# whwh747/A-Low-Texture-Robust-Hybrid-Feature-Based-Visual-Odometry

Hardware: AMD Instinct MI355X
Metric: RGB-D frames/sec (640×480, 1k ORB + LSD + PEAC) at 1/2/4/8 GPUs (higher is better)
Workload: dtype u8/u16 integer + f32/f64; 1 GPU; 640x480 synthetic RGB-D, 1000 ORB (quota; 3/4 std + 1/4 lowtex scenes) + LSD lines + PEAC planes, 8192 frames per GPU per step (std640); frames_per_gpu=8192, parallelism=frames sharded, 1 rank(s), no data-path collective, distinct_frames=256, resident_bytes_per_frame_estimate=21100000

## Files before the change

a-low-texture-robust-hybrid-feature-based-visual-odometry_amd/csrc/hvo_internal.hpp:

```cpp
#pragma once
#include <hip/hip_runtime.h>
#include <stdlib.h>
#include <stdint.h>
#include <string>
#include <vector>
#include "../../include/hvo.h"

#define HVO_MAX_LEVELS 16
#define HVO_EDGE_THRESHOLD 19
#define HVO_CELL_TILE 72
#define HVO_CELL_CAP 256
#define HVO_MAX_PROFILE 768
#define HVO_HAVE_PEAC 1
#define HVO_HAVE_LSD 1

struct LevelGeom {
    int w, h, pitch;
    int minBX, minBY, maxBX, maxBY;
    int nCols, nRows, wCell, hCell;
    int cell_off, ncells;
    int nfeat;
    int cand_off, cand_cap;
    int node_off, node_cap;
    int kp_off, kp_cap;
    int scaled_patch;
    float scale;
    unsigned long long img_off;
    unsigned long long lvl_off;
    int rs_off;
    int ry_off;
    int tile_off, ntx, nty;
};

struct CellDesc {
    short level, x0, y0, vw, vh, ox, oy, pad;
};

struct OrbTile {
    short bx0, by0, bw, bh;
    short fx0, fw;
    short cell;
    short dxa, dxb, dya, dyb;
    short pad[5];
};

struct OrbPlan {
    int w = 0, h = 0, nlevels = 0, batch = 0;
    LevelGeom lev[HVO_MAX_LEVELS];
    int ncells = 0, cand_total = 0, node_total = 0, kp_total = 0, ntiles = 0, max_cell = 0;
    size_t pyr_bytes = 0;
    size_t lvl_bytes = 0, blur_bytes = 0;
    int chunk = 0;
    bool resize_dw[HVO_MAX_LEVELS] = {};
    int last_chunks = 0;
    bool fused = false;
    int lt_off[HVO_MAX_LEVELS] = {}, lt_cnt[HVO_MAX_LEVELS] = {}, lt_tpw = 4;
    int lt_nw = 4;
    OrbTile *d_ltiles = nullptr;
    int2 *d_kpchunks = nullptr; int n_kpchunks = 0;
    int kp_cap = 0;
    LevelGeom *d_lev = nullptr;
    CellDesc *d_cells = nullptr;
    int *d_rs_xofs = nullptr; int *d_rs_xalpha = nullptr;
    int *d_rs_yofs = nullptr; int *d_rs_ybeta = nullptr;
    int4 *d_tiles = nullptr;
    uint8_t *d_pyr = nullptr, *d_blur = nullptr;
    uint8_t *d_lvl = nullptr, *d_lvl_base = nullptr;
    uint8_t *d_pyr_base = nullptr;
    uint32_t *d_cell_kp = nullptr; int *d_cell_cnt = nullptr;
    uint32_t *d_cand = nullptr; int *d_keys = nullptr, *d_keys_tmp = nullptr;
    int oct_slot_cap = 0;
    uint32_t *d_lvl_kp = nullptr; int *d_lvl_cnt = nullptr;
    hvo_keypoint *d_kp = nullptr; uint8_t *d_desc = nullptr; int *d_nkp = nullptr;
    int *d_flags = nullptr;
};

struct ProfileRec { const char *name; hipEvent_t e0, e1; float ms; bool used; hipStream_t st; };

struct Knob {
    bool set = false; int v = 0;
    void read(const char *name) { const char *e = getenv(name); set = e != nullptr; v = e ? atoi(e) : 0; }
    int or_(int dflt) const { return set ? v : dflt; }
    bool off() const { return set && v == 0; }
};
int hvo_ensure_dyn_lds(const void *kernel, size_t bytes);

struct hvo_ctx {
    hvo_params p;
    Knob kn_frame_perm, kn_upload_single;
    unsigned readings = 0;
    int device = 0;
    hipStream_t stream = nullptr;
    hipStream_t s_lsd = nullptr;
    hipStream_t s_peac = nullptr;
    hipEvent_t ev_lsd_pre = nullptr;
    bool lsd_pre_recorded = false;
    hipEvent_t ev_fast = nullptr;
    bool fast_recorded = false;
    int sched = 1;
    int sched_cfg = -1;
    bool orb_blur_late = false;
    uint8_t *d_stage_gray = nullptr; uint16_t *d_stage_depth = nullptr; size_t stage_gray_bytes = 0, stage_depth_bytes = 0;
    uint8_t *stage_gray_dst = nullptr; uint16_t *stage_depth_dst = nullptr;
    int stage_n = 0, stage_w = 0, stage_h = 0; bool stage_depth = false;
    hipStream_t s_stage_up = nullptr, s_stage_down = nullptr; hipEvent_t ev_stage_up = nullptr;
    char *d_result_slab = nullptr; size_t result_slab_bytes = 0;
    hipStream_t s_copy = nullptr; bool copy_hi = false;
    std::vector<std::pair<int, int *>> perms;
    double cull_dis = 5.0, cull_angle = 2.5, cull_endpoint = 15.0;
    bool last_cull = false;
    unsigned last_stages = 0;
    std::string last_error;
    OrbPlan orb;
    int umax[16];
    float scale[HVO_MAX_LEVELS], inv_scale[HVO_MAX_LEVELS];
    int nfeat[HVO_MAX_LEVELS];
    int8_t *d_pattern = nullptr; int *d_umax = nullptr;
    int batch_n = 0, batch_w = 0, batch_h = 0;
    bool have_depth = false;
    void *marena = nullptr;
    void *h_stage = nullptr; size_t h_stage_cap = 0;
    hipEvent_t ev_stage[2] = { nullptr, nullptr };
    bool profile = false;
    bool serialize = false;
    bool lsd_on_orb_stream = false;
    ProfileRec prof[HVO_MAX_PROFILE]; int nprof = 0;
    void *call_arena = nullptr; size_t call_arena_cap = 0;
    hipEvent_t po_ev[2] = { nullptr, nullptr }; float po_ms = 0.f;
    hipEvent_t ls_ev[3] = { nullptr, nullptr, nullptr }; float ls_ms[2] = { 0.f, 0.f };
    bool ls_batch_done = false;
    void *tail = nullptr;
    void *peac = nullptr;
    void *lsd = nullptr;
};

struct EdgeSel { unsigned s0, s1, s2; bool lo2; };
#ifdef __HIPCC__
static __device__ __forceinline__ EdgeSel edge_sel(int x0, int w)
{
    EdgeSel e; e.s0 = 0x03020100u; e.s1 = 0x07060504u; e.s2 = 0x07060504u;
    const int m = w - 1 - x0;
    e.lo2 = m <= 2;
    if (x0 >= 4 && m >= 7) return e;
    unsigned s0 = 0, s1 = 0, s2 = 0;
#pragma unroll
    for (int b = 0; b < 12; b++) {
        const int px = x0 - 4 + b;
        int r = px < 0 ? -px : (px >= w ? 2 * (w - 1) - px : px);
        int sb = r - (x0 - 4);
        if (b < 8) { if (sb < 0 || sb > 7) sb = b; }
        else if (e.lo2) { if (sb < 0 || sb > 7) sb = 7; }
        else { sb -= 4; if (sb < 0 || sb > 7) sb = b - 4; }
        if (b < 4) s0 |= (unsigned)sb << (8 * b);
        else if (b < 8) s1 |= (unsigned)sb << (8 * (b - 4));
        else s2 |= (unsigned)sb << (8 * (b - 8));
    }
    e.s0 = s0; e.s1 = s1; e.s2 = s2;
    return e;
}
static __device__ __forceinline__ void edge_fix(const EdgeSel &e, unsigned &W0, unsigned &W1, unsigned &W2)
{
    const unsigned a = e.lo2 ? W1 : W2, b = e.lo2 ? W0 : W1;
    const unsigned n0 = __builtin_amdgcn_perm(W1, W0, e.s0), n1 = __builtin_amdgcn_perm(W1, W0, e.s1);
    W2 = __builtin_amdgcn_perm(a, b, e.s2); W0 = n0; W1 = n1;
}
#endif

#define HVO_HIP(call)                                                                        \
    do {                                                                                     \
        hipError_t e_ = (call);                                                              \
        if (e_ != hipSuccess) {                                                              \
            ctx->last_error = std::string(#call) + ": " + hipGetErrorString(e_);            \
            return HVO_ERR_HIP;                                                              \
        }                                                                                    \
    } while (0)

static __device__ __forceinline__ double hvo_div_const(double a, double b, double y)
{
    const double q0 = a * y;
    const double q1 = fma(fma(-q0, b, a), y, q0);
    return fma(fma(-q1, b, a), y, q1);
}

static __device__ __forceinline__ float hvo_fatan2_deg(float y, float x)
{
    const float p1 = 0.9997878412794807f * (float)(180 / 3.14159265358979323846);
    const float p3 = -0.3258083974640975f * (float)(180 / 3.14159265358979323846);
    const float p5 = 0.1555786518463281f * (float)(180 / 3.14159265358979323846);
    const float p7 = -0.04432655554792128f * (float)(180 / 3.14159265358979323846);
    const float eps = (float)2.2204460492503131e-16;
    const float ax = fabsf(x), ay = fabsf(y);
    const bool hi = ax >= ay;
    const float c = __fdiv_rn(hi ? ay : ax, __fadd_rn(hi ? ax : ay, eps)), c2 = __fmul_rn(c, c);
    float r = __fmul_rn(__fadd_rn(__fmul_rn(__fadd_rn(__fmul_rn(__fadd_rn(__fmul_rn(p7, c2), p5), c2), p3), c2), p1), c);
    if (!hi) r = __fsub_rn(90.f, r);
    if (x < 0) r = __fsub_rn(180.f, r);
    if (y < 0) r = __fsub_rn(360.f, r);
// ... 201 lines not shown
```

a-low-texture-robust-hybrid-feature-based-visual-odometry_amd/csrc/orb_level.hip:

```cpp
#include "hvo_internal.hpp"
#include <string.h>
#include <algorithm>
#include <vector>

#define LT_TP 64
#define LT_ND (LT_TP / 4)
#define LT_TR 46
#define LT_MAXO 40
#define LT_CAND 368
#define LT_PEND 328
#define LT_TABN 48

typedef unsigned short lt_us2 __attribute__((ext_vector_type(2)));

struct __attribute__((aligned(16))) LtWave {
    uint32_t T[LT_TR * LT_ND];
    union {
        struct { uint8_t S[LT_TR * LT_TP]; unsigned short cand[LT_CAND]; unsigned short pend[LT_PEND]; unsigned long long mk_min[8], mk_ini[8]; } f;
        uint32_t V[((LT_TR + 1) / 2) * LT_MAXO];
    } u;
    int tab[4][LT_TABN];
};
static_assert(sizeof(LtWave) <= 8192, "five workgroups per CU");

struct LevelArgs {
    const uint8_t *rd; size_t rd_stride;
    uint8_t *wr; size_t wr_stride;
    uint8_t *blur; size_t blur_stride;
    LevelGeom L, D; int has_next;
    const OrbTile *tiles; int ntiles, tpw, groups, nframes;
    const int *xofs, *xalpha, *yofs, *ybeta;
    uint32_t *cell_kp; int *cell_cnt; int ncells, iniTh, minTh; int *flags;
    int k0, k1, k2, k3;
    int res_dw;
    int skip;
};

static __device__ __forceinline__ int lt_reflect(int p, int n)
{
    if (p < 0) p = -p;
    if (p >= n) p = 2 * (n - 1) - p;
    return p < 0 ? 0 : p;
}
static __device__ __forceinline__ int lt_mbcnt(unsigned long long m)
{
    return __builtin_amdgcn_mbcnt_hi((unsigned)(m >> 32), __builtin_amdgcn_mbcnt_lo((unsigned)m, 0u));
}

static __device__ __forceinline__ int lt_min3(int a, int b, int c) { int r; asm("v_min3_i32 %0, %1, %2, %3" : "=v"(r) : "v"(a), "v"(b), "v"(c)); return r; }
static __device__ __forceinline__ int lt_max3(int a, int b, int c) { int r; asm("v_max3_i32 %0, %1, %2, %3" : "=v"(r) : "v"(a), "v"(b), "v"(c)); return r; }

static __device__ __forceinline__ int lt_fast_score(const uint8_t *p, int v)
{
    constexpr int tp = LT_TP;
    int r[16];
    r[0] = p[3 * tp];    r[1] = p[3 * tp + 1];   r[2] = p[2 * tp + 2];   r[3] = p[tp + 3];
    r[4] = p[3];         r[5] = p[-tp + 3];      r[6] = p[-2 * tp + 2];  r[7] = p[-3 * tp + 1];
    r[8] = p[-3 * tp];   r[9] = p[-3 * tp - 1];  r[10] = p[-2 * tp - 2]; r[11] = p[-tp - 3];
    r[12] = p[-3];       r[13] = p[tp - 3];      r[14] = p[2 * tp - 2];  r[15] = p[3 * tp - 1];
    int d[16], e[16], a3[16], b3[16];
#pragma unroll
    for (int k = 0; k < 16; k++) { d[k] = v - r[k]; e[k] = r[k] - v; }
#pragma unroll
    for (int k = 0; k < 16; k++) { a3[k] = lt_min3(d[k], d[(k + 1) & 15], d[(k + 2) & 15]); b3[k] = lt_min3(e[k], e[(k + 1) & 15], e[(k + 2) & 15]); }
    int best = -1000;
#pragma unroll
    for (int k = 0; k < 16; k++)
        best = lt_max3(best, lt_min3(a3[k], a3[(k + 3) & 15], a3[(k + 6) & 15]), lt_min3(b3[k], b3[(k + 3) & 15], b3[(k + 6) & 15]));
    return best - 1;
}

static __device__ __forceinline__ void lt_row_sums(unsigned W0, unsigned W1, unsigned W2, unsigned klo, unsigned khi, unsigned hs[4])
{
    const unsigned A0 = __builtin_amdgcn_alignbyte(W1, W0, 1), B0 = __builtin_amdgcn_alignbyte(W2, W1, 1);
    const unsigned A1 = __builtin_amdgcn_alignbyte(W1, W0, 2), B1 = __builtin_amdgcn_alignbyte(W2, W1, 2);
    const unsigned A2 = __builtin_amdgcn_alignbyte(W1, W0, 3), B2 = __builtin_amdgcn_alignbyte(W2, W1, 3);
    hs[0] = __builtin_amdgcn_udot4(A0, klo, __builtin_amdgcn_udot4(B0, khi, 0u, false), false);
    hs[1] = __builtin_amdgcn_udot4(A1, klo, __builtin_amdgcn_udot4(B1, khi, 0u, false), false);
    hs[2] = __builtin_amdgcn_udot4(A2, klo, __builtin_amdgcn_udot4(B2, khi, 0u, false), false);
    hs[3] = __builtin_amdgcn_udot4(W1, klo, __builtin_amdgcn_udot4(W2, khi, 0u, false), false);
}
static __device__ __forceinline__ unsigned lt_dot2(unsigned a, unsigned w, unsigned c)
{
    return __builtin_amdgcn_udot2(__builtin_bit_cast(lt_us2, a), __builtin_bit_cast(lt_us2, w), c, false);
}

template <int NW>
__global__ __launch_bounds__(64 * NW, 5) void k_orb_level(const LevelArgs A)
{
    __shared__ LtWave lds_[NW];
    const int wv = threadIdx.x >> 6, lane = threadIdx.x & 63;
    const int xcd = blockIdx.x & 7, q = blockIdx.x >> 3;
    const int fr8 = q / A.groups, g = q - fr8 * A.groups;
    const int frame = fr8 * 8 + xcd;
    if (frame >= A.nframes) return;
    LtWave &W = lds_[wv];
    const LevelGeom &L = A.L;
    const uint8_t *img = A.rd + (size_t)frame * A.rd_stride;
    uint8_t *bdst = A.blur + (size_t)frame * A.blur_stride;
    const uint8_t *T8 = reinterpret_cast<const uint8_t *>(W.T);
    const unsigned long long ltm = (1ull << lane) - 1ull;

    for (int ti = 0; ti < A.tpw; ti++) {
        const int tidx = (g * A.tpw + ti) * NW + wv;
        if (tidx >= A.ntiles) break;
        const OrbTile t = A.tiles[tidx];
        const int lx0 = t.bx0 - 4, ly0 = t.by0 - 3;
        const int rows = t.bh + 6;
        const int xr = max(t.fx0 + t.fw, t.bx0 + t.bw) + 3;
        __builtin_amdgcn_wave_barrier();
        {
            typedef uint32_t lt_u4 __attribute__((ext_vector_type(4), aligned(4)));
            uint4 v[3];
#pragma unroll
            for (int k = 0; k < 3; k++) {
                const int i = lane + 64 * k, r = i >> 2, c = i & 3;
                v[k] = make_uint4(0, 0, 0, 0);
                if (r < rows) {
                    const int y = lt_reflect(ly0 + r, L.h);
                    const lt_u4 q4 = *reinterpret_cast<const lt_u4 *>(img + (size_t)y * L.pitch + lx0 + 16 * c);
                    v[k] = make_uint4(q4.x, q4.y, q4.z, q4.w);
                }
            }
            int tb0 = 0, tb1 = 0, tb2 = 0, tb3 = 0;
            const bool want_tab = A.has_next && lane < LT_TABN;
            if (want_tab) {
                const int dx = min(t.dxa + lane, A.D.w - 1), dy = min(t.dya + lane, A.D.h - 1);
                tb0 = A.xofs[dx]; tb1 = A.xalpha[dx]; tb2 = A.yofs[dy]; tb3 = A.ybeta[dy];
            }
#pragma unroll
            for (int k = 0; k < 3; k++) {
                const int i = lane + 64 * k;
                if ((i >> 2) < rows) reinterpret_cast<uint4 *>(W.T)[i] = v[k];
            }
            if (want_tab) { W.tab[0][lane] = tb0; W.tab[1][lane] = tb1; W.tab[2][lane] = tb2; W.tab[3][lane] = tb3; }
        }
        if (lx0 < 0) {
            if (lane < rows) { const unsigned d1 = W.T[lane * LT_ND + 1]; W.T[lane * LT_ND] = __builtin_amdgcn_perm(d1, d1, 0x01020300u); }
        }
        if (xr > L.w) {
            uint8_t *Tb = reinterpret_cast<uint8_t *>(W.T);
            if (lane < rows) {
                const int c = L.w - lx0;
#pragma unroll
                for (int k = 0; k < 3; k++) if (L.w + k < xr) Tb[lane * LT_TP + c + k] = Tb[lane * LT_TP + c - 2 - k];
            }
        }
        __builtin_amdgcn_wave_barrier();

        if (t.fw > 0 && !(A.skip & 1)) {
            uint8_t *S = W.u.f.S;
            {
                uint4 *Sz = reinterpret_cast<uint4 *>(S);
                const int nz = (rows * LT_TP + 15) >> 4;
                for (int i = lane; i < nz; i += 64) Sz[i] = make_uint4(0, 0, 0, 0);
            }
            const int cx0 = t.fx0 - lx0, cx1 = cx0 + t.fw, ih = t.bh, iw = t.fw, P = iw * ih;
            const int dws = cx0 >> 2, nd = ((cx1 - 1) >> 2) - dws + 1, items = ih * nd;
            const int rcp = (65536 + nd - 1) / nd;
            const int minTh = A.minTh;
            int ncand = 0, npend = 0;
            auto rest = [&](const unsigned short *pp, int cnt) {
                int pass = 0, xy = 0;
                if (lane < cnt) {
                    xy = pp[lane];
                    const uint8_t *qq = T8 + (xy >> 8) * LT_TP + (xy & 0xFF);
                    const int v = qq[0];
#define LT_PMN(o) min((int)qq[o], (int)qq[-(o)])
#define LT_PMX(o) max((int)qq[o], (int)qq[-(o)])
                    const int n0 = LT_PMN(3 * LT_TP), n1 = LT_PMN(3), n2 = LT_PMN(2 * LT_TP + 2), n3 = LT_PMN(-2 * LT_TP + 2);
                    const int n4 = LT_PMN(3 * LT_TP + 1), n5 = LT_PMN(LT_TP + 3), n6 = LT_PMN(-LT_TP + 3), n7 = LT_PMN(-3 * LT_TP + 1);
                    const int x0 = LT_PMX(3 * LT_TP), x1 = LT_PMX(3), x2 = LT_PMX(2 * LT_TP + 2), x3 = LT_PMX(-2 * LT_TP + 2);
                    const int x4 = LT_PMX(3 * LT_TP + 1), x5 = LT_PMX(LT_TP + 3), x6 = LT_PMX(-LT_TP + 3), x7 = LT_PMX(-3 * LT_TP + 1);
#undef LT_PMN
#undef LT_PMX
                    const int M1 = lt_max3(lt_max3(n0, n1, n2), lt_max3(n3, n4, n5), max(n6, n7));
                    const int M2 = lt_min3(lt_min3(x0, x1, x2), lt_min3(x3, x4, x5), min(x6, x7));
                    pass = (int)(M1 < v - minTh) | (int)(M2 > v + minTh);
                }
                const unsigned long long m = __ballot(pass != 0);
                const int p = ncand + __popcll(m & ltm);
                if (pass && p < LT_CAND) W.u.f.cand[p] = (unsigned short)xy;
                ncand += __popcll(m);
            };
            for (int base = 0; base < items; base += 64) {
                const int it = base + lane;
                const int ok = it < items;
                const int itc = ok ? it : 0;
                const int r = (itc * rcp) >> 16, dwi = dws + itc - r * nd;
                const unsigned t4 = W.T[r * LT_ND + dwi], v4 = W.T[(r + 3) * LT_ND + dwi], b4 = W.T[(r + 6) * LT_ND + dwi];
                const int xb = 4 * dwi;
                const int jl = max(cx0 - xb, 0), jh = min(cx1 - xb, 4);
                const unsigned inm = ok ? (((1u << jh) - 1u) & ~((1u << jl) - 1u)) : 0u;
                int pj[4];
#pragma unroll
                for (int j = 0; j < 4; j++) {
                    const int v = (v4 >> (8 * j)) & 0xFF, tt = (t4 >> (8 * j)) & 0xFF, bb = (b4 >> (8 * j)) & 0xFF;
                    pj[j] = (int)((inm >> j) & 1u) & ((int)(min(tt, bb) < v - minTh) | (int)(max(tt, bb) > v + minTh));
                }
                const unsigned long long m0 = __ballot(pj[0] != 0), m1 = __ballot(pj[1] != 0), m2 = __ballot(pj[2] != 0), m3 = __ballot(pj[3] != 0);
                if ((m0 | m1 | m2 | m3) != 0ull) {
                    const int p0 = npend + lt_mbcnt(m0) + lt_mbcnt(m1) + lt_mbcnt(m2) + lt_mbcnt(m3);
                    const int p1 = p0 + pj[0], p2 = p1 + pj[1], p3 = p2 + pj[2];
                    const int yx = ((r + 3) << 8) | xb;
                    W.u.f.pend[pj[0] ? p0 : LT_PEND - 1] = (unsigned short)yx;
                    W.u.f.pend[pj[1] ? p1 : LT_PEND - 1] = (unsigned short)(yx + 1);
                    W.u.f.pend[pj[2] ? p2 : LT_PEND - 1] = (unsigned short)(yx + 2);
                    W.u.f.pend[pj[3] ? p3 : LT_PEND - 1] = (unsigned short)(yx + 3);
                    npend += __popcll(m0) + __popcll(m1) + __popcll(m2) + __popcll(m3);
                    int head = 0;
                    while (npend - head >= 64) { rest(W.u.f.pend + head, 64); head += 64; }
                    if (head) {
                        const int left = npend - head;
                        const int tv = W.u.f.pend[head + (lane < left ? lane : 0)];
                        if (lane < left) W.u.f.pend[lane] = (unsigned short)tv;
                        npend = left;
                    }
                }
            }
            if (npend > 0) rest(W.u.f.pend, npend);
            __builtin_amdgcn_wave_barrier();
            const uint8_t *T0 = T8 + 3 * LT_TP + cx0;
            uint8_t *S0 = S + 3 * LT_TP + cx0;
            if (ncand <= LT_CAND) {
                for (int i = lane; i < ncand; i += 64) {
                    const int xy = W.u.f.cand[i], o = (xy >> 8) * LT_TP + (xy & 0xFF);
                    const int s = lt_fast_score(T8 + o, T8[o]);
                    S[o] = (uint8_t)(s >= minTh ? s : 0);
                }
            } else {
                for (int p = lane; p < P; p += 64) {
                    const int y = p / iw, x = p - y * iw;
                    const int s = lt_fast_score(T0 + y * LT_TP + x, T0[y * LT_TP + x]);
                    S0[y * LT_TP + x] = (uint8_t)(s >= minTh ? s : 0);
                }
            }
            __builtin_amdgcn_wave_barrier();
            uint32_t *out = A.cell_kp + ((size_t)frame * A.ncells + t.cell) * HVO_CELL_CAP;
            const int ex = lx0 - L.minBX, ey = ly0 - L.minBY;
            int n_ini = 0, pos = 0;
            if (ncand <= LT_CAND) {
                int st = 0;
                for (int base = 0; base < ncand; base += 64, st++) {
                    const int i = base + lane;
                    bool okk = false; int v = 0;
                    if (i < ncand) {
                        const int xy = W.u.f.cand[i];
                        const uint8_t *sp = S + (xy >> 8) * LT_TP + (xy & 0xFF);
                        v = sp[0];
                        const int nb = lt_max3(lt_max3(sp[-1], sp[1], sp[-LT_TP - 1]), lt_max3(sp[-LT_TP], sp[-LT_TP + 1], sp[LT_TP - 1]), max((int)sp[LT_TP], (int)sp[LT_TP + 1]));
                        okk = (v != 0) & (v > nb);
                    }
                    const unsigned long long mm = __ballot(okk), mi = __ballot(okk & (v >= A.iniTh));
                    n_ini += __popcll(mi);
                    if (lane == 0) { W.u.f.mk_min[st] = mm; W.u.f.mk_ini[st] = mi; }
                }
                __builtin_amdgcn_wave_barrier();
                const bool use_ini = n_ini > 0;
                st = 0;
                for (int base = 0; base < ncand; base += 64, st++) {
                    const unsigned long long m = use_ini ? W.u.f.mk_ini[st] : W.u.f.mk_min[st];
                    if (m) {
                        if ((m >> lane) & 1ull) {
                            const int xy = W.u.f.cand[base + lane], x = xy & 0xFF, y = xy >> 8;
                            const int p = pos + __popcll(m & ltm);
                            if (p < HVO_CELL_CAP) out[p] = (uint32_t)(x + ex) | ((uint32_t)(y + ey) << 12) | ((uint32_t)S[y * LT_TP + x] << 24);
                        }
                        pos += __popcll(m);
                    }
                }
            } else {
                for (int pass = 0; pass < 2; pass++) {
                    const bool use_ini = n_ini > 0;
                    for (int p0 = 0; p0 < P; p0 += 64) {
                        const int p = p0 + lane;
                        bool okk = false; int v = 0, x = 0, y = 0;
                        if (p < P) {
                            y = p / iw; x = p - y * iw;
                            const uint8_t *sp = S0 + y * LT_TP + x;
                            v = sp[0];
                            const int nb = lt_max3(lt_max3(sp[-1], sp[1], sp[-LT_TP - 1]), lt_max3(sp[-LT_TP], sp[-LT_TP + 1], sp[LT_TP - 1]), max((int)sp[LT_TP], (int)sp[LT_TP + 1]));
                            okk = (v != 0) & (v > nb);
                        }
                        if (pass == 0) n_ini += __popcll(__ballot(okk && v >= A.iniTh));
                        else {
                            const bool em = okk && (!use_ini || v >= A.iniTh);
                            const unsigned long long m = __ballot(em);
                            if (em) {
                                const int pp = pos + __popcll(m & ltm);
                                if (pp < HVO_CELL_CAP) out[pp] = (uint32_t)(x + cx0 + ex) | ((uint32_t)(y + 3 + ey) << 12) | ((uint32_t)v << 24);
                            }
                            pos += __popcll(m);
                        }
                    }
                }
            }
            if (lane == 0) {
                if (pos > HVO_CELL_CAP) { atomicOr(&A.flags[frame], 1); pos = HVO_CELL_CAP; }
                A.cell_cnt[(size_t)frame * A.ncells + t.cell] = pos;
            }
            __builtin_amdgcn_wave_barrier();
        }

        const int nbd = t.bw >> 2;
        if (nbd > 0 && !(A.skip & 2)) {
            const unsigned klo = (unsigned)A.k0 | ((unsigned)A.k1 << 8) | ((unsigned)A.k2 << 16) | ((unsigned)A.k3 << 24);
            const unsigned khi = (unsigned)A.k2 | ((unsigned)A.k1 << 8) | ((unsigned)A.k0 << 16);
            const int np = (rows + 1) >> 1;
            const int rcpb = (65536 + nbd - 1) / nbd;
            for (int it = lane; it < np * nbd; it += 64) {
                const int p = (it * rcpb) >> 16, o = it - p * nbd;
                const int r0 = 2 * p, r1 = min(2 * p + 1, rows - 1);
                const uint32_t *ra = W.T + r0 * LT_ND + o, *rb = W.T + r1 * LT_ND + o;
                unsigned ha[4], hb[4];
                lt_row_sums(ra[0], ra[1], ra[2], klo, khi, ha);
                lt_row_sums(rb[0], rb[1], rb[2], klo, khi, hb);
                *reinterpret_cast<uint4 *>(W.u.V + p * LT_MAXO + 4 * o) =
                    make_uint4(ha[0] | (hb[0] << 16), ha[1] | (hb[1] << 16), ha[2] | (hb[2] << 16), ha[3] | (hb[3] << 16));
            }
            __builtin_amdgcn_wave_barrier();
            const unsigned k01 = (unsigned)A.k0 | ((unsigned)A.k1 << 16), k23 = (unsigned)A.k2 | ((unsigned)A.k3 << 16);
            const unsigned k21 = (unsigned)A.k2 | ((unsigned)A.k1 << 16), k0_ = (unsigned)A.k0;
            const unsigned k_0 = (unsigned)A.k0 << 16, k12 = (unsigned)A.k1 | ((unsigned)A.k2 << 16);
            const unsigned k32 = (unsigned)A.k3 | ((unsigned)A.k2 << 16), k10 = (unsigned)A.k1 | ((unsigned)A.k0 << 16);
            const int nq = (t.bh + 1) >> 1;
            const int wv4 = L.w & ~3;
            for (int it = lane; it < nq * nbd; it += 64) {
                const int qq = (it * rcpb) >> 16, o = it - qq * nbd;
                const uint4 P0 = *reinterpret_cast<const uint4 *>(W.u.V + qq * LT_MAXO + 4 * o);
                const uint4 P1 = *reinterpret_cast<const uint4 *>(W.u.V + (qq + 1) * LT_MAXO + 4 * o);
                const uint4 P2 = *reinterpret_cast<const uint4 *>(W.u.V + (qq + 2) * LT_MAXO + 4 * o);
                const uint4 P3 = *reinterpret_cast<const uint4 *>(W.u.V + (qq + 3) * LT_MAXO + 4 * o);
                const unsigned p0[4] = { P0.x, P0.y, P0.z, P0.w }, p1[4] = { P1.x, P1.y, P1.z, P1.w };
                const unsigned p2[4] = { P2.x, P2.y, P2.z, P2.w }, p3[4] = { P3.x, P3.y, P3.z, P3.w };
                const int x0 = t.bx0 + 4 * o;
                const unsigned halfup = x0 >= wv4 ? 1u : 0u;
                unsigned ta[4], tb[4];
#pragma unroll
                for (int j = 0; j < 4; j++) {
                    const unsigned s0 = lt_dot2(p0[j], k01, lt_dot2(p1[j], k23, lt_dot2(p2[j], k21, lt_dot2(p3[j], k0_, 0u))));
                    const unsigned s1 = lt_dot2(p0[j], k_0, lt_dot2(p1[j], k12, lt_dot2(p2[j], k32, lt_dot2(p3[j], k10, 0u))));
                    ta[j] = min(s0 + 32767u + (((s0 >> 16) & 1u) | halfup), 0x00FFFFFFu);
                    tb[j] = min(s1 + 32767u + (((s1 >> 16) & 1u) | halfup), 0x00FFFFFFu);
                }
                const unsigned oa = __builtin_amdgcn_perm(__builtin_amdgcn_perm(ta[3], ta[2], 0x0c0c0602u), __builtin_amdgcn_perm(ta[1], ta[0], 0x0c0c0602u), 0x05040100u);
                const unsigned ob = __builtin_amdgcn_perm(__builtin_amdgcn_perm(tb[3], tb[2], 0x0c0c0602u), __builtin_amdgcn_perm(tb[1], tb[0], 0x0c0c0602u), 0x05040100u);
                const int y = t.by0 + 2 * qq;
                *reinterpret_cast<uint32_t *>(bdst + (size_t)y * L.pitch + x0) = oa;
                if (2 * qq + 1 < t.bh) *reinterpret_cast<uint32_t *>(bdst + (size_t)(y + 1) * L.pitch + x0) = ob;
            }
        }

        if (A.has_next && t.dxb > t.dxa && t.dyb > t.dya && !(A.skip & 4)) {
            const LevelGeom &D = A.D;
            uint8_t *dst = A.wr + (size_t)frame * A.wr_stride;
            const int dd0 = t.dxa >> 2, ndd = (t.dxb - t.dxa) >> 2;
            const int nr = t.dyb - t.dya;
            constexpr int RG = 4;
            const int ngr = (nr + RG - 1) / RG;
            const int rcpd = (65536 + ndd - 1) / ndd;
            for (int it = lane; it < ngr * ndd; it += 64) {
                const int gr = (it * rcpd) >> 16, c = it - gr * ndd;
                const int dxq = 4 * (dd0 + c);
                int sxo[4]; unsigned a01[4];
#pragma unroll
                for (int i = 0; i < 4; i++) {
                    sxo[i] = W.tab[0][4 * c + i] - lx0;
                    a01[i] = (unsigned)W.tab[1][4 * c + i];
                }
                const int wbase = sxo[0] >> 2;
                unsigned sel = 0;
#pragma unroll
                for (int i = 0; i < 4; i++) sel |= (unsigned)((sxo[i] - 4 * wbase) & 7) << (8 * i);
                auto hrow = [&](int sy, unsigned tt[4]) {
                    if (A.res_dw) {
                        const uint32_t *rp = W.T + (sy - ly0) * LT_ND + wbase;
                        const uint32_t w0 = rp[0], w1 = rp[1], w2 = rp[2];
                        const uint32_t Lb = __builtin_amdgcn_perm(w1, w0, sel);
                        const uint32_t Rb = __builtin_amdgcn_perm(__builtin_amdgcn_alignbyte(w2, w1, 1), __builtin_amdgcn_alignbyte(w1, w0, 1), sel);
                        tt[0] = lt_dot2(__builtin_amdgcn_perm(Rb, Lb, 0x0c040c00u), a01[0], 0u);
                        tt[1] = lt_dot2(__builtin_amdgcn_perm(Rb, Lb, 0x0c050c01u), a01[1], 0u);
                        tt[2] = lt_dot2(__builtin_amdgcn_perm(Rb, Lb, 0x0c060c02u), a01[2], 0u);
                        tt[3] = lt_dot2(__builtin_amdgcn_perm(Rb, Lb, 0x0c070c03u), a01[3], 0u);
                    } else {
                        const uint8_t *rp = T8 + (sy - ly0) * LT_TP;
#pragma unroll
                        for (int i = 0; i < 4; i++) {
                            const int sx = min(max(sxo[i], 0), LT_TP - 2);
                            tt[i] = lt_dot2((unsigned)rp[sx] | ((unsigned)rp[sx + 1] << 16), a01[i], 0u);
                        }
                    }
                };
#pragma unroll
                for (int rr = 0; rr < RG; rr++) {
                    const int dyu = t.dya + gr * RG + rr, dy = min(dyu, t.dyb - 1);
                    const int yo = W.tab[2][dy - t.dya], sy0 = yo & 0xFFFF, sy1 = yo >> 16;
                    const unsigned yb = (unsigned)W.tab[3][dy - t.dya];
                    const unsigned b0 = yb & 0xFFFFu, b1 = yb >> 16;
                    unsigned t0[4], t1[4];
                    hrow(sy0, t0);
                    hrow(sy1, t1);
                    uint32_t ov = 0;
#pragma unroll
                    for (int i = 0; i < 4; i++) {
                        const unsigned v = ((__umul24(b0, t0[i] >> 4) >> 16) + (__umul24(b1, t1[i] >> 4) >> 16) + 2u) >> 2;
                        ov |= (v & 0xFFu) << (8 * i);
                    }
                    if (dyu < t.dyb) *reinterpret_cast<uint32_t *>(dst + (size_t)dy * D.pitch + dxq) = ov;
                }
            }
        }
    }
}

struct LtIv { int a, b, idx; };

static void lt_split(std::vector<LtIv> &v, int a, int b, int align)
{
    if (b <= a) return;
    const int len = b - a, n = (len + LT_MAXO - 1) / LT_MAXO;
    int step = (len + n - 1) / n;
    step = (step + align - 1) / align * align;
    for (int s = a; s < b; s += step) v.push_back({ s, std::min(s + step, b), -1 });
}

bool orb_level_build(OrbPlan &P, const std::vector<CellDesc> &cells, const std::vector<int> &xofs, const std::vector<int> &yofs, std::vector<OrbTile> &tiles)
{
    tiles.clear();
    for (int l = 0; l < P.nlevels; l++) {
        LevelGeom &L = P.lev[l];
        P.lt_off[l] = (int)tiles.size();
        std::vector<LtIv> cols, rws;
        for (int c = L.cell_off; c < L.cell_off + L.ncells; c++) {
            const CellDesc &cd = cells[c];
            const int fx = cd.x0 + 3, fxe = cd.x0 + cd.vw - 3, fy = cd.y0 + 3, fye = cd.y0 + cd.vh - 3;
            bool hc = false, hr = false;
            for (auto &iv : cols) hc |= iv.a == fx;
            for (auto &iv : rws) hr |= iv.a == fy;
            if (!hc) cols.push_back({ fx, fxe, (int)cols.size() });
            if (!hr) rws.push_back({ fy, fye, (int)rws.size() });
        }
        if ((int)(cols.size() * rws.size()) != L.ncells) return false;
        for (size_t j = 1; j < cols.size(); j++) if (cols[j].a != cols[j - 1].b) return false;
        for (size_t i = 1; i < rws.size(); i++) if (rws[i].a != rws[i - 1].b) return false;
        const int W4 = (L.w + 3) & ~3;
        std::vector<LtIv> xs, ys;
        if (cols.empty()) { lt_split(xs, 0, W4, 4); lt_split(ys, 0, L.h, 1); }
        else {
            lt_split(xs, 0, cols[0].a & ~3, 4);
            for (size_t j = 0; j < cols.size(); j++) {
                const int a = cols[j].a & ~3, b = (j + 1 < cols.size() ? cols[j + 1].a : cols[j].b) & ~3;
                xs.push_back({ a, b, (int)j });
            }
            lt_split(xs, cols.back().b & ~3, W4, 4);
            lt_split(ys, 0, rws[0].a, 1);
            for (size_t i = 0; i < rws.size(); i++) ys.push_back({ rws[i].a, rws[i].b, (int)i });
            lt_split(ys, rws.back().b, L.h, 1);
        }
        const bool has_next = l + 1 < P.nlevels;
        const int *xo = has_next ? xofs.data() + P.lev[l + 1].rs_off : nullptr;
        const int *yo = has_next ? yofs.data() + P.lev[l + 1].ry_off : nullptr;
        const int dw = has_next ? P.lev[l + 1].w : 0, dh = has_next ? P.lev[l + 1].h : 0;
        for (auto &iy : ys) for (auto &ix : xs) {
            OrbTile t; memset(&t, 0, sizeof(t));
            t.bx0 = (short)ix.a; t.bw = (short)(ix.b - ix.a); t.by0 = (short)iy.a; t.bh = (short)(iy.b - iy.a);
            t.cell = -1; t.fx0 = (short)ix.a; t.fw = 0;
            if (ix.idx >= 0 && iy.idx >= 0) {
                t.fx0 = (short)cols[ix.idx].a; t.fw = (short)(cols[ix.idx].b - cols[ix.idx].a);
                t.cell = (short)(L.cell_off + iy.idx * (int)cols.size() + ix.idx);
                const CellDesc &cd = cells[t.cell];
                if (cd.x0 + 3 != t.fx0 || cd.y0 + 3 != t.by0 || cd.vh - 6 != t.bh || cd.vw - 6 != t.fw) return false;
            }
            if (t.bh < 1 || (t.bw < 1 && t.fw < 1)) continue;
            const int xr = std::max(t.fx0 + t.fw, t.bx0 + t.bw) + 3;
            if (t.bw > LT_MAXO || t.bh > LT_MAXO || t.bh + 6 > LT_TR || xr - (t.bx0 - 4) > LT_TP || (t.bw & 3) || (t.bx0 & 3)) return false;
            if (t.fw > 0 && ((t.fw * t.bh + 3) / 4 > LT_CAND + 1000)) return false;
            int dxa = 0, dxb = 0, dya = 0, dyb = 0;
            if (has_next && t.bw > 0) {
                const int dw4 = (dw + 3) & ~3;
                while (dxa < dw4 && xo[std::min(dxa, dw - 1)] < t.bx0) dxa += 4;
                dxb = dxa; while (dxb < dw4 && xo[std::min(dxb, dw - 1)] < t.bx0 + t.bw) dxb += 4;
                while (dya < dh && (yo[dya] & 0xFFFF) < t.by0) dya++;
                dyb = dya; while (dyb < dh && (yo[dyb] & 0xFFFF) < t.by0 + t.bh) dyb++;
                for (int dx = dxa; dx < std::min(dxb, dw); dx++) if (xo[dx] + 1 - (t.bx0 - 4) > LT_TP - 1) return false;
            }
            if (dxb - dxa > LT_TABN || dyb - dya > LT_TABN) return false;
            t.dxa = (short)dxa; t.dxb = (short)dxb; t.dya = (short)dya; t.dyb = (short)dyb;
            tiles.push_back(t);
        }
        P.lt_cnt[l] = (int)tiles.size() - P.lt_off[l];
    }
    return true;
}

int orb_level_run(hvo_ctx *ctx, int c0, int n, hipStream_t st, int k0, int k1, int k2, int k3)
{
    OrbPlan &P = ctx->orb;
    for (int l = 0; l < P.nlevels; l++) {
        LevelArgs A;
        A.L = P.lev[l]; A.has_next = l + 1 < P.nlevels; A.D = P.lev[A.has_next ? l + 1 : l];
        if (l == 0) { A.rd = P.d_pyr + (size_t)c0 * P.pyr_bytes; A.rd_stride = P.pyr_bytes; } else { A.rd = P.d_lvl + A.L.lvl_off; A.rd_stride = P.lvl_bytes; }
        A.wr = P.d_lvl + A.D.lvl_off; A.wr_stride = P.lvl_bytes;
        A.blur = P.d_blur + A.L.img_off; A.blur_stride = P.blur_bytes;
        A.tiles = P.d_ltiles + P.lt_off[l]; A.ntiles = P.lt_cnt[l];
        const int nw = P.lt_nw;
        A.tpw = P.lt_tpw; A.groups = (A.ntiles + nw * A.tpw - 1) / (nw * A.tpw); A.nframes = n;
        A.xofs = P.d_rs_xofs + A.D.rs_off; A.xalpha = P.d_rs_xalpha + A.D.rs_off; A.yofs = P.d_rs_yofs + A.D.ry_off; A.ybeta = P.d_rs_ybeta + A.D.ry_off;
        A.cell_kp = P.d_cell_kp; A.cell_cnt = P.d_cell_cnt; A.ncells = P.ncells; A.iniTh = ctx->p.orb_ini_th_fast; A.minTh = ctx->p.orb_min_th_fast;
        A.res_dw = A.has_next && P.resize_dw[l + 1];
#ifdef HVO_TIMING_KNOBS
        A.skip = getenv("HVO_LT_SKIP") ? atoi(getenv("HVO_LT_SKIP")) : 0;
#else
        A.skip = 0;
#endif
        if (ctx->readings & HVO_READING_BLUR_FLOAT) A.skip |= 2;
        A.flags = P.d_flags + c0; A.k0 = k0; A.k1 = k1; A.k2 = k2; A.k3 = k3;
        if (A.ntiles < 1) continue;
        const int n8 = (n + 7) / 8 * 8;
        if (nw == 1) hipLaunchKernelGGL(k_orb_level<1>, dim3((unsigned)(n8 * A.groups)), dim3(64), 0, st, A);
        else if (nw == 2) hipLaunchKernelGGL(k_orb_level<2>, dim3((unsigned)(n8 * A.groups)), dim3(128), 0, st, A);
        else hipLaunchKernelGGL(k_orb_level<4>, dim3((unsigned)(n8 * A.groups)), dim3(256), 0, st, A);
    }
    return HVO_OK;
}
```

Baseline: 55980 frames/s.

## Precompute per-tile reciprocals and row grouping, rebalance ORB level kernel lane work

Moves per-tile reciprocal divisions and the resize row-group size into host-side tile planning, where a cost model picks the row group per tile. The tile descriptor is loaded as scalar dwords via readfirstlane, and resize offset tables are pre-biased to LDS byte offsets. Blur loops split the trailing partial wave so both 32-lane halves each compute one output row instead of leaving half the wave idle. Skip knobs are compiled out unless a timing macro is defined. These cut per-lane integer division and VALU waste at the cost of more complex indexing and a tighter tile plan that can now reject tiles.

```diff
diff --git a/a-low-texture-robust-hybrid-feature-based-visual-odometry_amd/csrc/hvo_internal.hpp b/a-low-texture-robust-hybrid-feature-based-visual-odometry_amd/csrc/hvo_internal.hpp
--- a/a-low-texture-robust-hybrid-feature-based-visual-odometry_amd/csrc/hvo_internal.hpp
+++ b/a-low-texture-robust-hybrid-feature-based-visual-odometry_amd/csrc/hvo_internal.hpp
@@ -41,8 +41,11 @@
     short fx0, fw;
     short cell;
     short dxa, dxb, dya, dyb;
-    short pad[5];
-};
+    unsigned short rcpf, rcpb, rcpd;
+    unsigned char rg, ngr;
+    short pad;
+};
+static_assert(sizeof(OrbTile) == 32, "k_orb_level reads a tile as eight dwords");
 
 struct OrbPlan {
     int w = 0, h = 0, nlevels = 0, batch = 0;
diff --git a/a-low-texture-robust-hybrid-feature-based-visual-odometry_amd/csrc/orb_level.hip b/a-low-texture-robust-hybrid-feature-based-visual-odometry_amd/csrc/orb_level.hip
--- a/a-low-texture-robust-hybrid-feature-based-visual-odometry_amd/csrc/orb_level.hip
+++ b/a-low-texture-robust-hybrid-feature-based-visual-odometry_amd/csrc/orb_level.hip
@@ -12,6 +12,12 @@
 #define LT_TABN 48
 
 typedef unsigned short lt_us2 __attribute__((ext_vector_type(2)));
+
+#ifdef HVO_TIMING_KNOBS
+#define LT_SKIP(b) (A.skip & (b))
+#else
+#define LT_SKIP(b) 0
+#endif
 
 struct __attribute__((aligned(16))) LtWave {
     uint32_t T[LT_TR * LT_ND];
@@ -89,22 +95,31 @@
 __global__ __launch_bounds__(64 * NW, 5) void k_orb_level(const LevelArgs A)
 {
     __shared__ LtWave lds_[NW];
-    const int wv = threadIdx.x >> 6, lane = threadIdx.x & 63;
+    const int wv = __builtin_amdgcn_readfirstlane((int)(threadIdx.x >> 6)), lane = threadIdx.x & 63;
     const int xcd = blockIdx.x & 7, q = blockIdx.x >> 3;
     const int fr8 = q / A.groups, g = q - fr8 * A.groups;
     const int frame = fr8 * 8 + xcd;
     if (frame >= A.nframes) return;
+    int frame_v = frame;
+    asm("" : "+v"(frame_v));
     LtWave &W = lds_[wv];
     const LevelGeom &L = A.L;
-    const uint8_t *img = A.rd + (size_t)frame * A.rd_stride;
-    uint8_t *bdst = A.blur + (size_t)frame * A.blur_stride;
+    const uint8_t *img = A.rd + (size_t)frame_v * A.rd_stride;
+    uint8_t *bdst = A.blur + (size_t)frame_v * A.blur_stride;
     const uint8_t *T8 = reinterpret_cast<const uint8_t *>(W.T);
     const unsigned long long ltm = (1ull << lane) - 1ull;
 
     for (int ti = 0; ti < A.tpw; ti++) {
         const int tidx = (g * A.tpw + ti) * NW + wv;
         if (tidx >= A.ntiles) break;
-        const OrbTile t = A.tiles[tidx];
+        OrbTile t;
+        {
+            const uint32_t *tq = reinterpret_cast<const uint32_t *>(A.tiles + tidx);
+            uint32_t tw[8];
+#pragma unroll
+            for (int k = 0; k < 8; k++) tw[k] = __builtin_amdgcn_readfirstlane(tq[k]);
+            memcpy(&t, tw, sizeof(t));
+        }
         const int lx0 = t.bx0 - 4, ly0 = t.by0 - 3;
         const int rows = t.bh + 6;
         const int xr = max(t.fx0 + t.fw, t.bx0 + t.bw) + 3;
@@ -127,6 +142,8 @@
             if (want_tab) {
                 const int dx = min(t.dxa + lane, A.D.w - 1), dy = min(t.dya + lane, A.D.h - 1);
                 tb0 = A.xofs[dx]; tb1 = A.xalpha[dx]; tb2 = A.yofs[dy]; tb3 = A.ybeta[dy];
+                tb0 -= lx0;
+                tb2 = (int)(((unsigned)(((tb2 & 0xFFFF) - ly0) * LT_TP) & 0xFFFFu) | ((unsigned)(((tb2 >> 16) - ly0) * LT_TP) << 16));
             }
 #pragma unroll
             for (int k = 0; k < 3; k++) {
@@ -148,7 +165,7 @@
         }
         __builtin_amdgcn_wave_barrier();
 
-        if (t.fw > 0 && !(A.skip & 1)) {
+        if (t.fw > 0 && !LT_SKIP(1)) {
             uint8_t *S = W.u.f.S;
             {
                 uint4 *Sz = reinterpret_cast<uint4 *>(S);
@@ -157,7 +174,7 @@
             }
             const int cx0 = t.fx0 - lx0, cx1 = cx0 + t.fw, ih = t.bh, iw = t.fw, P = iw * ih;
             const int dws = cx0 >> 2, nd = ((cx1 - 1) >> 2) - dws + 1, items = ih * nd;
-            const int rcp = (65536 + nd - 1) / nd;
+            const int rcp = t.rcpf + 1;
             const int minTh = A.minTh;
             int ncand = 0, npend = 0;
             auto rest = [&](const unsigned short *pp, int cnt) {
@@ -236,7 +253,7 @@
                 }
             }
             __builtin_amdgcn_wave_barrier();
-            uint32_t *out = A.cell_kp + ((size_t)frame * A.ncells + t.cell) * HVO_CELL_CAP;
+            uint32_t *out = A.cell_kp + ((size_t)frame_v * A.ncells + t.cell) * HVO_CELL_CAP;
             const int ex = lx0 - L.minBX, ey = ly0 - L.minBY;
             int n_ini = 0, pos = 0;
             if (ncand <= LT_CAND) {
@@ -296,8 +313,8 @@
                 }
             }
             if (lane == 0) {
-                if (pos > HVO_CELL_CAP) { atomicOr(&A.flags[frame], 1); pos = HVO_CELL_CAP; }
-                A.cell_cnt[(size_t)frame * A.ncells + t.cell] = pos;
+                if (pos > HVO_CELL_CAP) { atomicOr(&A.flags[frame_v], 1); pos = HVO_CELL_CAP; }
+                A.cell_cnt[(size_t)frame_v * A.ncells + t.cell] = pos;
             }
             __builtin_amdgcn_wave_barrier();
         }
@@ -306,107 +323,146 @@
         if (nbd > 0 && !(A.skip & 2)) {
             const unsigned klo = (unsigned)A.k0 | ((unsigned)A.k1 << 8) | ((unsigned)A.k2 << 16) | ((unsigned)A.k3 << 24);
             const unsigned khi = (unsigned)A.k2 | ((unsigned)A.k1 << 8) | ((unsigned)A.k0 << 16);
-            const int np = (rows + 1) >> 1;
-            const int rcpb = (65536 + nbd - 1) / nbd;
-            for (int it = lane; it < np * nbd; it += 64) {
+            typedef unsigned short __attribute__((may_alias)) lt_u16a;
+            const int np = (rows + 1) >> 1, nrow = np * nbd;
+            const int rcpb = t.rcpb + 1;
+            const int hh = lane >> 5, l32 = lane & 31;
+            const int remr = nrow & 63, endr = remr > 32 ? nrow : nrow - remr;
+            for (int base = 0; base < endr; base += 64) {
+                const int it = base + lane;
+                if (it < endr) {
+                    const int p = (it * rcpb) >> 16, o = it - p * nbd;
+                    const int r0 = 2 * p, r1 = min(2 * p + 1, rows - 1);
+                    const uint32_t *ra = W.T + r0 * LT_ND + o, *rb = W.T + r1 * LT_ND + o;
+                    unsigned ha[4], hb[4];
+                    lt_row_sums(ra[0], ra[1], ra[2], klo, khi, ha);
+                    lt_row_sums(rb[0], rb[1], rb[2], klo, khi, hb);
+                    *reinterpret_cast<uint4 *>(W.u.V + p * LT_MAXO + 4 * o) =
+                        make_uint4(ha[0] | (hb[0] << 16), ha[1] | (hb[1] << 16), ha[2] | (hb[2] << 16), ha[3] | (hb[3] << 16));
+                }
+            }
+            if (endr < nrow && l32 < remr) {
+                const int it = endr + l32;
                 const int p = (it * rcpb) >> 16, o = it - p * nbd;
-                const int r0 = 2 * p, r1 = min(2 * p + 1, rows - 1);
-                const uint32_t *ra = W.T + r0 * LT_ND + o, *rb = W.T + r1 * LT_ND + o;
-                unsigned ha[4], hb[4];
+                const uint32_t *ra = W.T + min(2 * p + hh, rows - 1) * LT_ND + o;
+                unsigned ha[4];
                 lt_row_sums(ra[0], ra[1], ra[2], klo, khi, ha);
-                lt_row_sums(rb[0], rb[1], rb[2], klo, khi, hb);
-                *reinterpret_cast<uint4 *>(W.u.V + p * LT_MAXO + 4 * o) =
-                    make_uint4(ha[0] | (hb[0] << 16), ha[1] | (hb[1] << 16), ha[2] | (hb[2] << 16), ha[3] | (hb[3] << 16));
+                lt_u16a *vp = reinterpret_cast<lt_u16a *>(W.u.V + p * LT_MAXO + 4 * o) + hh;
+                vp[0] = (unsigned short)ha[0]; vp[2] = (unsigned short)ha[1]; vp[4] = (unsigned short)ha[2]; vp[6] = (unsigned short)ha[3];
             }
             __builtin_amdgcn_wave_barrier();
-            const unsigned k01 = (unsigned)A.k0 | ((unsigned)A.k1 << 16), k23 = (unsigned)A.k2 | ((unsigned)A.k3 << 16);
-            const unsigned k21 = (unsigned)A.k2 | ((unsigned)A.k1 << 16), k0_ = (unsigned)A.k0;
-            const unsigned k_0 = (unsigned)A.k0 << 16, k12 = (unsigned)A.k1 | ((unsigned)A.k2 << 16);
-            const unsigned k32 = (unsigned)A.k3 | ((unsigned)A.k2 << 16), k10 = (unsigned)A.k1 | ((unsigned)A.k0 << 16);
-            const int nq = (t.bh + 1) >> 1;
+            unsigned k01 = (unsigned)A.k0 | ((unsigned)A.k1 << 16), k23 = (unsigned)A.k2 | ((unsigned)A.k3 << 16);
+            unsigned k21 = (unsigned)A.k2 | ((unsigned)A.k1 << 16), k0_ = (unsigned)A.k0;
+            unsigned k_0 = (unsigned)A.k0 << 16, k12 = (unsigned)A.k1 | ((unsigned)A.k2 << 16);
+            unsigned k32 = (unsigned)A.k3 | ((unsigned)A.k2 << 16), k10 = (unsigned)A.k1 | ((unsigned)A.k0 << 16);
+            const int nq = (t.bh + 1) >> 1, ncol = nq * nbd;
             const int wv4 = L.w & ~3;
-            for (int it = lane; it < nq * nbd; it += 64) {
+            auto quot = [](unsigned s, unsigned halfup) { return min(s + 32767u + (((s >> 16) & 1u) | halfup), 0x00FFFFFFu); };
+            auto pack4 = [](const unsigned q[4]) {
+                return __builtin_amdgcn_perm(__builtin_amdgcn_perm(q[3], q[2], 0x0c0c0602u), __builtin_amdgcn_perm(q[1], q[0], 0x0c0c0602u), 0x05040100u);
+            };
+            const int remc = ncol & 63, endc = remc > 32 ? ncol : ncol - remc;
+            for (int base = 0; base < endc; base += 64) {
+                const int it = base + lane;
+                if (it < endc) {
+                    const int qq = (it * rcpb) >> 16, o = it - qq * nbd;
+                    const uint4 P0 = *reinterpret_cast<const uint4 *>(W.u.V + qq * LT_MAXO + 4 * o);
+                    const uint4 P1 = *reinterpret_cast<const uint4 *>(W.u.V + (qq + 1) * LT_MAXO + 4 * o);
+                    const uint4 P2 = *reinterpret_cast<const uint4 *>(W.u.V + (qq + 2) * LT_MAXO + 4 * o);
+                    const uint4 P3 = *reinterpret_cast<const uint4 *>(W.u.V + (qq + 3) * LT_MAXO + 4 * o);
+                    const unsigned p0[4] = { P0.x, P0.y, P0.z, P0.w }, p1[4] = { P1.x, P1.y, P1.z, P1.w };
+                    const unsigned p2[4] = { P2.x, P2.y, P2.z, P2.w }, p3[4] = { P3.x, P3.y, P3.z, P3.w };
+                    const int x0 = t.bx0 + 4 * o;
+                    const unsigned halfup = x0 >= wv4 ? 1u : 0u;
+                    unsigned ta[4], tb[4];
+#pragma unroll
+                    for (int j = 0; j < 4; j++) {
+                        ta[j] = quot(lt_dot2(p0[j], k01, lt_dot2(p1[j], k23, lt_dot2(p2[j], k21, lt_dot2(p3[j], k0_, 0u)))), halfup);
+                        tb[j] = quot(lt_dot2(p0[j], k_0, lt_dot2(p1[j], k12, lt_dot2(p2[j], k32, lt_dot2(p3[j], k10, 0u)))), halfup);
+                    }
+                    const int y = t.by0 + 2 * qq;
+                    *reinterpret_cast<uint32_t *>(bdst + (size_t)y * L.pitch + x0) = pack4(ta);
+                    if (2 * qq + 1 < t.bh) *reinterpret_cast<uint32_t *>(bdst + (size_t)(y + 1) * L.pitch + x0) = pack4(tb);
+                }
+            }
+            if (endc < ncol && l32 < remc) {
+                const int it = endc + l32;
                 const int qq = (it * rcpb) >> 16, o = it - qq * nbd;
-                const uint4 P0 = *reinterpret_cast<const uint4 *>(W.u.V + qq * LT_MAXO + 4 * o);
-                const uint4 P1 = *reinterpret_cast<const uint4 *>(W.u.V + (qq + 1) * LT_MAXO + 4 * o);
-                const uint4 P2 = *reinterpret_cast<const uint4 *>(W.u.V + (qq + 2) * LT_MAXO + 4 * o);
-                const uint4 P3 = *reinterpret_cast<const uint4 *>(W.u.V + (qq + 3) * LT_MAXO + 4 * o);
-                const unsigned p0[4] = { P0.x, P0.y, P0.z, P0.w }, p1[4] = { P1.x, P1.y, P1.z, P1.w };
-                const unsigned p2[4] = { P2.x, P2.y, P2.z, P2.w }, p3[4] = { P3.x, P3.y, P3.z, P3.w };
-                const int x0 = t.bx0 + 4 * o;
-                const unsigned halfup = x0 >= wv4 ? 1u : 0u;
-                unsigned ta[4], tb[4];
-#pragma unroll
-                for (int j = 0; j < 4; j++) {
-                    const unsigned s0 = lt_dot2(p0[j], k01, lt_dot2(p1[j], k23, lt_dot2(p2[j], k21, lt_dot2(p3[j], k0_, 0u))));
-                    const unsigned s1 = lt_dot2(p0[j], k_0, lt_dot2(p1[j], k12, lt_dot2(p2[j], k32, lt_dot2(p3[j], k10, 0u))));
-                    ta[j] = min(s0 + 32767u + (((s0 >> 16) & 1u) | halfup), 0x00FFFFFFu);
-                    tb[j] = min(s1 + 32767u + (((s1 >> 16) & 1u) | halfup), 0x00FFFFFFu);
-                }
-                const unsigned oa = __builtin_amdgcn_perm(__builtin_amdgcn_perm(ta[3], ta[2], 0x0c0c0602u), __builtin_amdgcn_perm(ta[1], ta[0], 0x0c0c0602u), 0x05040100u);
-                const unsigned ob = __builtin_amdgcn_perm(__builtin_amdgcn_perm(tb[3], tb[2], 0x0c0c0602u), __builtin_amdgcn_perm(tb[1], tb[0], 0x0c0c0602u), 0x05040100u);
-                const int y = t.by0 + 2 * qq;
-                *reinterpret_cast<uint32_t *>(bdst + (size_t)y * L.pitch + x0) = oa;
-                if (2 * qq + 1 < t.bh) *reinterpret_cast<uint32_t *>(bdst + (size_t)(y + 1) * L.pitch + x0) = ob;
-            }
-        }
-
-        if (A.has_next && t.dxb > t.dxa && t.dyb > t.dya && !(A.skip & 4)) {
+                if (2 * qq + hh < t.bh) {
+                    const uint4 P0 = *reinterpret_cast<const uint4 *>(W.u.V + qq * LT_MAXO + 4 * o);
+                    const uint4 P1 = *reinterpret_cast<const uint4 *>(W.u.V + (qq + 1) * LT_MAXO + 4 * o);
+                    const uint4 P2 = *reinterpret_cast<const uint4 *>(W.u.V + (qq + 2) * LT_MAXO + 4 * o);
+                    const uint4 P3 = *reinterpret_cast<const uint4 *>(W.u.V + (qq + 3) * LT_MAXO + 4 * o);
+                    const unsigned p0[4] = { P0.x, P0.y, P0.z, P0.w }, p1[4] = { P1.x, P1.y, P1.z, P1.w };
+                    const unsigned p2[4] = { P2.x, P2.y, P2.z, P2.w }, p3[4] = { P3.x, P3.y, P3.z, P3.w };
+                    const unsigned ka = hh ? k_0 : k01, kb = hh ? k12 : k23, kc = hh ? k32 : k21, kd = hh ? k10 : k0_;
+                    const int x0 = t.bx0 + 4 * o;
+                    const unsigned halfup = x0 >= wv4 ? 1u : 0u;
+                    unsigned ta[4];
+#pragma unroll
+                    for (int j = 0; j < 4; j++) ta[j] = quot(lt_dot2(p0[j], ka, lt_dot2(p1[j], kb, lt_dot2(p2[j], kc, lt_dot2(p3[j], kd, 0u)))), halfup);
+                    *reinterpret_cast<uint32_t *>(bdst + (size_t)(t.by0 + 2 * qq + hh) * L.pitch + x0) = pack4(ta);
+                }
+            }
+        }
+
+        if (A.has_next && t.dxb > t.dxa && t.dyb > t.dya && !LT_SKIP(4)) {
             const LevelGeom &D = A.D;
-            uint8_t *dst = A.wr + (size_t)frame * A.wr_stride;
+            uint8_t *dst = A.wr + (size_t)frame_v * A.wr_stride;
             const int dd0 = t.dxa >> 2, ndd = (t.dxb - t.dxa) >> 2;
             const int nr = t.dyb - t.dya;
-            constexpr int RG = 4;
-            const int ngr = (nr + RG - 1) / RG;
-            const int rcpd = (65536 + ndd - 1) / ndd;
-            for (int it = lane; it < ngr * ndd; it += 64) {
-                const int gr = (it * rcpd) >> 16, c = it - gr * ndd;
-                const int dxq = 4 * (dd0 + c);
-                int sxo[4]; unsigned a01[4];
-#pragma unroll
-                for (int i = 0; i < 4; i++) {
-                    sxo[i] = W.tab[0][4 * c + i] - lx0;
-                    a01[i] = (unsigned)W.tab[1][4 * c + i];
-                }
-                const int wbase = sxo[0] >> 2;
-                unsigned sel = 0;
-#pragma unroll
-                for (int i = 0; i < 4; i++) sel |= (unsigned)((sxo[i] - 4 * wbase) & 7) << (8 * i);
-                auto hrow = [&](int sy, unsigned tt[4]) {
-                    if (A.res_dw) {
-                        const uint32_t *rp = W.T + (sy - ly0) * LT_ND + wbase;
-                        const uint32_t w0 = rp[0], w1 = rp[1], w2 = rp[2];
-                        const uint32_t Lb = __builtin_amdgcn_perm(w1, w0, sel);
-                        const uint32_t Rb = __builtin_amdgcn_perm(__builtin_amdgcn_alignbyte(w2, w1, 1), __builtin_amdgcn_alignbyte(w1, w0, 1), sel);
-                        tt[0] = lt_dot2(__builtin_amdgcn_perm(Rb, Lb, 0x0c040c00u), a01[0], 0u);
-                        tt[1] = lt_dot2(__builtin_amdgcn_perm(Rb, Lb, 0x0c050c01u), a01[1], 0u);
-                        tt[2] = lt_dot2(__builtin_amdgcn_perm(Rb, Lb, 0x0c060c02u), a01[2], 0u);
-                        tt[3] = lt_dot2(__builtin_amdgcn_perm(Rb, Lb, 0x0c070c03u), a01[3], 0u);
-                    } else {
-                        const uint8_t *rp = T8 + (sy - ly0) * LT_TP;
+            const int rg = t.rg, nit = t.ngr * ndd;
+            const int rcpd = t.rcpd + 1;
+            for (int base = 0; base < nit; base += 64) {
+                const int it = base + lane;
+                if (it < nit) {
+                    const int gr = (it * rcpd) >> 16, c = it - gr * ndd;
+                    int sxo[4]; unsigned a01[4];
+#pragma unroll
+                    for (int i = 0; i < 4; i++) {
+                        sxo[i] = W.tab[0][4 * c + i];
+                        a01[i] = (unsigned)W.tab[1][4 * c + i];
+                    }
+                    const int wbase = sxo[0] >> 2;
+                    unsigned sel = 0;
+#pragma unroll
+                    for (int i = 0; i < 4; i++) sel |= (unsigned)((sxo[i] - 4 * wbase) & 7) << (8 * i);
+                    auto hrow = [&](int ro, unsigned tt[4]) {
+                        if (A.res_dw) {
+                            const uint32_t *rp = reinterpret_cast<const uint32_t *>(T8 + ro) + wbase;
+                            const uint32_t w0 = rp[0], w1 = rp[1], w2 = rp[2];
+                            const uint32_t Lb = __builtin_amdgcn_perm(w1, w0, sel);
+                            const uint32_t Rb = __builtin_amdgcn_perm(__builtin_amdgcn_alignbyte(w2, w1, 1), __builtin_amdgcn_alignbyte(w1, w0, 1), sel);
+                            tt[0] = lt_dot2(__builtin_amdgcn_perm(Rb, Lb, 0x0c040c00u), a01[0], 0u);
+                            tt[1] = lt_dot2(__builtin_amdgcn_perm(Rb, Lb, 0x0c050c01u), a01[1], 0u);
+                            tt[2] = lt_dot2(__builtin_amdgcn_perm(Rb, Lb, 0x0c060c02u), a01[2], 0u);
+                            tt[3] = lt_dot2(__builtin_amdgcn_perm(Rb, Lb, 0x0c070c03u), a01[3], 0u);
+                        } else {
+                            const uint8_t *rp = T8 + ro;
+#pragma unroll
+                            for (int i = 0; i < 4; i++) {
+                                const int sx = min(max(sxo[i], 0), LT_TP - 2);
+                                tt[i] = lt_dot2((unsigned)rp[sx] | ((unsigned)rp[sx + 1] << 16), a01[i], 0u);
+                            }
+                        }
+                    };
+                    int row = gr * rg;
+                    uint8_t *dp = dst + (size_t)(t.dya + row) * D.pitch + 4 * (dd0 + c);
+                    for (int rr = 0; rr < rg; rr++, row++, dp += D.pitch) {
+                        const int rc = min(row, nr - 1);
+                        const unsigned yo = (unsigned)W.tab[2][rc], yb = (unsigned)W.tab[3][rc];
+                        const unsigned b0 = yb & 0xFFFFu, b1 = yb >> 16;
+                        unsigned t0[4], t1[4];
+                        hrow((int)(yo & 0xFFFFu), t0);
+                        hrow((int)(yo >> 16), t1);
+                        uint32_t ov = 0;
 #pragma unroll
                         for (int i = 0; i < 4; i++) {
-                            const int sx = min(max(sxo[i], 0), LT_TP - 2);
-                            tt[i] = lt_dot2((unsigned)rp[sx] | ((unsigned)rp[sx + 1] << 16), a01[i], 0u);
+                            const unsigned v = ((__umul24(b0, t0[i] >> 4) >> 16) + (__umul24(b1, t1[i] >> 4) >> 16) + 2u) >> 2;
+                            ov |= (v & 0xFFu) << (8 * i);
                         }
-                    }
-                };
-#pragma unroll
-                for (int rr = 0; rr < RG; rr++) {
-                    const int dyu = t.dya + gr * RG + rr, dy = min(dyu, t.dyb - 1);
-                    const int yo = W.tab[2][dy - t.dya], sy0 = yo & 0xFFFF, sy1 = yo >> 16;
-                    const unsigned yb = (unsigned)W.tab[3][dy - t.dya];
-                    const unsigned b0 = yb & 0xFFFFu, b1 = yb >> 16;
-                    unsigned t0[4], t1[4];
-                    hrow(sy0, t0);
-                    hrow(sy1, t1);
-                    uint32_t ov = 0;
-#pragma unroll
-                    for (int i = 0; i < 4; i++) {
-                        const unsigned v = ((__umul24(b0, t0[i] >> 4) >> 16) + (__umul24(b1, t1[i] >> 4) >> 16) + 2u) >> 2;
-                        ov |= (v & 0xFFu) << (8 * i);
-                    }
-                    if (dyu < t.dyb) *reinterpret_cast<uint32_t *>(dst + (size_t)dy * D.pitch + dxq) = ov;
+                        if (row < nr) *reinterpret_cast<uint32_t *>(dp) = ov;
+                    }
                 }
             }
         }
@@ -486,6 +542,20 @@
             }
             if (dxb - dxa > LT_TABN || dyb - dya > LT_TABN) return false;
             t.dxa = (short)dxa; t.dxb = (short)dxb; t.dya = (short)dya; t.dyb = (short)dyb;
+            auto rcp16 = [](int n) { return (unsigned short)(n > 0 ? (65536 + n - 1) / n - 1 : 0); };
+            if (t.fw > 0) { const int cx0 = t.fx0 - (t.bx0 - 4); t.rcpf = rcp16(((cx0 + t.fw - 1) >> 2) - (cx0 >> 2) + 1); }
+            t.rcpb = rcp16(t.bw >> 2); t.rcpd = rcp16((dxb - dxa) >> 2);
+            const int nr = dyb - dya, ndd = (dxb - dxa) >> 2;
+            t.rg = 1; t.ngr = 0;
+            if (nr > 0 && ndd > 0) {
+                long best = -1;
+                for (int rg = 1; rg <= nr; rg++) {
+                    const int ngr = (nr + rg - 1) / rg;
+                    const long cost = (long)((ngr * ndd + 63) / 64) * (24 + 84 * rg);
+                    if (best < 0 || cost < best) { best = cost; t.rg = (unsigned char)rg; t.ngr = (unsigned char)ngr; }
+                }
+                if (t.rg * t.ngr < nr || (t.ngr - 1) * t.rg >= nr) return false;
+            }
             tiles.push_back(t);
         }
         P.lt_cnt[l] = (int)tiles.size() - P.lt_off[l];
```

Measured after the change: 56490 frames/s, median of 6. About the same (+0.9%).
